# RohanVKashyap/resolution-pde

Hardware: AMD Instinct MI355X
Metric: training samples/sec, FFNO2D NS 256^2 (higher is better)
Workload: dtype f32; 1 GPU; FFNO2D(1,1,width=64,n_layers=4,n_modes=20,factor=4,ff_weight_norm,n_ff_layers=3,layer_norm,dropout=0.1) train step on [B,1,256,256] Gaussian random fields (BASELINE configs[2]); batch_per_gpu=32, global_batch=32, optimizer=AdamW lr=1e-3 (rpde.optim.FlatAdamW: torch.optim.AdamW's rule, one kernel), parallelism=single, grad_bucket_bytes=6828576, target=input advanced by a fixed spectral filter (utils/synthetic.py:advance)

## Files before the change

### resolution-pde_amd/csrc/feedforward.hip

```cpp
#include "rpde_internal.h"
#include "pointwise.h"
#include "gemm_kernel.h"
#include "ff_fused.h"
#include "wgrad_h2.h"
#include "thin_linear.h"
#include "conv_small.h"

#include <vector>

namespace rpde {


static inline int ff_in(const rpde_ff_params* p, int l) { return l == 0 ? p->dim : p->dim * p->factor; }
static inline int ff_out(const rpde_ff_params* p, int l) { return l == p->n_layers - 1 ? p->dim : p->dim * p->factor; }

static inline int wgrad_split(long P, int out_f, int in_f) {
  const int tiles = ((out_f + 127) / 128) * ((in_f + 127) / 128);
  long s = 768 / tiles;
  const long cap = (P + 127) / 128;
  if (s > cap) s = cap;
  if (s < 1) s = 1;
  if (s > 1024) s = 1024;
  return (int)s;
}

static inline bool worth_presplit(long P, int n, int k) { return P >= 1024 && k % 32 == 0 && n > 32; }
static int linear_fwd_impl(const float* x, const float* w, const float* b, float* y, long P, int in_f, int out_f,
                           int act_out, float* dy, float drop_p, uint64_t drop_seed, hipStream_t st,
                           void* wimg = nullptr, const uint64_t* drop_epoch = nullptr, bool wimg_ready = false) {
  if (act_out == RPDE_ACT_IDENTITY && !dy && drop_p == 0.f) {
    if (in_f <= 4 && thin_linear_ok(in_f, out_f) && al16(y)) return thin_expand(x, w, in_f, 1, b, y, P, in_f, out_f, st);
    if (out_f <= 4 && thin_linear_ok(out_f, in_f) && al16(x)) return thin_contract(x, w, in_f, 1, b, y, P, out_f, in_f, st);
  }
  rpde_gemm_desc d = gemm_desc();
  d.A = x; d.a_kmajor = 1; d.lda = in_f;
  d.B = w; d.b_kmajor = 1; d.ldb = in_f;
  if (wimg && worth_presplit(P, out_f, in_f)) {
    if (!wimg_ready) RPDE_TRY(split_weights(w, 1, in_f, out_f, in_f, wimg, st));
    d.b_split = wimg;
  }
  d.C = y; d.ldc = out_f;
  d.M = (int)P; d.N = out_f; d.K = in_f;
  d.bias = b; d.bias_mode = b ? 1 : 0;
  d.write_act = act_out; d.aux_out = act_out ? dy : nullptr;
  if (act_out) { d.drop_p = drop_p; d.drop_seed = drop_seed; d.drop_ld = out_f; d.drop_where = 4; d.drop_epoch = drop_epoch; }
  return launch_gemm(d, st);
}

static int linear_wgrad_impl(const float* x, const float* gy, float* gw, float* gb, long P, int in_f, int out_f,
                             float* ws_slabs, float* ws_colsum, hipStream_t st, int act_x = RPDE_ACT_IDENTITY,
                             FoldJobs* defer = nullptr) {
  if (act_x == RPDE_ACT_IDENTITY && (gw || gb)) {
    if (in_f <= 4 && thin_linear_ok(in_f, out_f) && al16(gy)) return thin_outer(x, gy, gw, 1, gb, nullptr, P, in_f, out_f, ws_slabs, st);
    if (out_f <= 4 && thin_linear_ok(out_f, in_f) && al16(x)) return thin_outer(gy, x, gw, 0, nullptr, gb, P, out_f, in_f, ws_slabs, st);
  }
  if (gw && wgrad_h2_ok(P, out_f, in_f)) {
    RPDE_TRY(wgrad_h2(gy, x, gw, P, in_f, out_f, act_x, ws_slabs, st, defer));
  } else if (gw) {
    const int S = wgrad_split(P, out_f, in_f);
    rpde_gemm_desc d = gemm_desc();
    d.A = gy; d.a_kmajor = 0; d.lda = out_f;
    d.B = x; d.b_kmajor = 0; d.ldb = in_f; d.act_b = act_x;
    d.M = out_f; d.N = in_f; d.K = (int)P;
    if (S > 1) {
      d.C = ws_slabs; d.ldc = in_f; d.ksplit = S; d.sCk = (long)out_f * in_f;
      RPDE_TRY(launch_gemm(d, st));
      if (!(defer && defer->add(ws_slabs, gw, out_f * in_f, S, (long)out_f * in_f)))
        RPDE_TRY(reduce_slabs(ws_slabs, gw, (long)out_f * in_f, S, (long)out_f * in_f, 1.f, 0, st));
    } else {
      d.C = gw; d.ldc = in_f;
      RPDE_TRY(launch_gemm(d, st));
    }
  }
  if (gb) RPDE_TRY(colsum(gy, gb, P, out_f, out_f, ws_colsum, 0, st));
  return RPDE_OK;
}

static inline long colsum_tiles(long P) { return (P + 127) / 128; }
static inline bool can_fuse_colsum(const float* gy, const float* w, const float* gx, const float* z, long P, int in_f,
                                   int out_f) {
  return P > 64 && in_f % 4 == 0 && out_f % 4 == 0 && al16(gy) && al16(w) && al16(gx) && (!z || al16(z));
}

static int linear_dgrad_impl(const float* gy, const float* w, float* gx, long P, int in_f, int out_f,
                             const float* dstored, float* colsum_slab, hipStream_t st, void* wimg = nullptr,
                             bool wimg_ready = false) {
// ... 89 lines not shown
  RPDE_CHECK_ARG(p && prep, "feedforward_prepare: bad arguments");
  Arena ar(prep, prep_bytes);
  const FfFusedImg f(ar);
  RPDE_CHECK_ARG(ff3_fused_ok(p, 32) && ar.ok(), "feedforward_prepare: shape not fused or buffer too small");
  RPDE_CHECK_ARG(p->weights && p->weights[0] && p->weights[1] && p->weights[2], "feedforward_prepare: null weights");
  return ff3_fused_prepare(p, f.img, as_stream(stream));
}

int rpde_feedforward_fwd_prepared(const rpde_ff_params* p, const float* x, const float* residual, float* out, int64_t P,
                                  const void* prep, size_t prep_bytes, void* stream) {
  RPDE_CHECK_ARG(p && x && out && prep && P > 0 && P < (1L << 31), "feedforward_fwd_prepared: bad arguments");
  Arena ar(const_cast<void*>(prep), prep_bytes);
  const FfFusedImg f(ar);
  RPDE_CHECK_ARG(ff3_fused_ok(p, P) && ar.ok(), "feedforward_fwd_prepared: shape not fused");
  RPDE_CHECK_ARG(!p->layer_norm || (p->ln_gamma && p->ln_beta), "feedforward_fwd_prepared: layer_norm needs gamma/beta");
  RPDE_CHECK_ARG(p->dropout_p == 0.f, "feedforward_fwd_prepared: evaluation only");
  return ff3_fused_fwd(p, x, residual, nullptr, nullptr, out , out, P,
                       f.img, as_stream(stream), true);
}

int rpde_feedforward_fwd(const rpde_ff_params* p, const float* x, const float* residual, float* const* hs,
                         float* const* ds, float* z_last, float* out, int64_t P, void* ws, size_t ws_bytes, void* stream) {
  RPDE_CHECK_ARG(p && x && z_last && out && P > 0, "feedforward_fwd: bad arguments");
  RPDE_CHECK_ARG(p->n_layers >= 1 && p->dim > 0 && p->factor > 0, "feedforward_fwd: bad shape");
  RPDE_CHECK_ARG(P < (1L << 31), "feedforward_fwd: too many points for one call");
  RPDE_CHECK_ARG(p->dropout_p >= 0.f && p->dropout_p < 1.f, "feedforward_fwd: dropout %f", p->dropout_p);
  hipStream_t st = as_stream(stream);
  Arena far(ws, ws_bytes);
  const FfFusedImg fused(far);
  if (ff3_fused_ok(p, P) && far.ok()) {
    RPDE_CHECK_ARG(p->weights[0] && p->weights[1] && p->weights[2], "feedforward_fwd: null weights");
    RPDE_CHECK_ARG(!p->layer_norm || (p->ln_gamma && p->ln_beta), "feedforward_fwd: layer_norm needs gamma/beta");
    return ff3_fused_fwd(p, x, residual, hs, ds, z_last, out, P, fused.img, st);
  }
  RPDE_CHECK_ARG(p->n_layers == 1 || hs, "feedforward_fwd: hidden buffers missing");
  const int L = p->n_layers;
  Arena ar(ws, ws_bytes);
  bool all_imgs = ws != nullptr && L <= SplitJobs::MAX;
  const FfFwdImgs imgs(ar, *p, all_imgs ? L : 1);
  all_imgs = all_imgs && ar.ok();
  float* const* wimg = imgs.wimg.data();
  if (all_imgs) {
    SplitJobs sj;
    for (int l = 0; l < L; ++l) {
      RPDE_CHECK_ARG(p->weights[l], "feedforward_fwd: null layer %d weight", l);
      if (worth_presplit(P, ff_out(p, l), ff_in(p, l))) sj.add(p->weights[l], 1, ff_in(p, l), ff_out(p, l), ff_in(p, l), wimg[l]);
    }
    RPDE_TRY(split_weights_multi(sj, st));
  }
  for (int l = 0; l < L; ++l) {
    const bool last = l == L - 1;
    RPDE_CHECK_ARG(p->weights[l] && (last || hs[l]), "feedforward_fwd: null layer %d buffers", l);
    const float* in = l == 0 ? x : hs[l - 1];
    RPDE_TRY(linear_fwd_impl(in, p->weights[l], p->biases ? p->biases[l] : nullptr, last ? z_last : hs[l], P, ff_in(p, l),
                             ff_out(p, l), last ? RPDE_ACT_IDENTITY : RPDE_ACT_GELU, (last || !ds) ? nullptr : ds[l],
                             p->dropout_p, layer_seed(p->seed, l), st, all_imgs ? wimg[l] : wimg[0], p->seed_epoch, all_imgs));
  }
  return ff_tail_fwd(z_last, residual, out, P, p->dim, p->layer_norm, p->ln_eps, p->ln_gamma, p->ln_beta,
                     make_drop(p->dropout_p, layer_seed(p->seed, L - 1), p->seed_epoch), p->post_act, st);
}

int rpde_feedforward_bwd(const rpde_ff_params* p, const float* x, const float* const* hs, const float* const* ds,
                         const float* z_last, const float* grad_out, float* grad_x, float* const* grad_weights,
                         float* const* grad_biases, float* grad_gamma, float* grad_beta, int64_t P, void* ws,
                         size_t ws_bytes, void* stream) {
  RPDE_CHECK_ARG(p && x && z_last && grad_out && P > 0, "feedforward_bwd: bad arguments");
  RPDE_CHECK_ARG(P < (1L << 31), "feedforward_bwd: too many points for one call");
  const int L = p->n_layers;
  const int hid = ff_hid(*p);
  const bool fused = ff3_fused_ok(p, P) && hs && hs[0] && hs[1];
  RPDE_CHECK_ARG(p->n_layers == 1 || (hs && (ds || fused)), "feedforward_bwd: saved hidden tensors missing");
  RPDE_CARVE("feedforward_bwd", FfBwdWork, wk, ws, ws_bytes, *p, P, fused);
  hipStream_t st = as_stream(stream);
  float *buf0 = wk.buf0, *buf1 = wk.buf1, *small = wk.small, *tailws = wk.tailws;
  const std::vector<float*>&slabs_l = wk.slabs, &csum_l = wk.csum, &wt_l = wk.wt;
  void* wt = wt_l[0];

  if (fused) {
    const int recompute = !(ds && ds[0] && ds[1]);
    const int act_h = recompute ? RPDE_ACT_GELU : RPDE_ACT_IDENTITY;
    float *dz3 = wk.dz3, *part = wk.part;
    void* fimg = wk.fimg;
    int grid = 0;
    RPDE_TRY(ff3_fused_bwd_launch(p, recompute ? hs : ds, recompute, z_last, grad_out, dz3, buf0, buf1, nullptr, part, &grid, P,
                                  fimg, st));
    const bool both = grad_x && grad_weights && wgrad_h2_dgrad_ok(P, hid, p->dim);
    if (grad_x && !both) RPDE_TRY(linear_dgrad_impl(buf1, p->weights[0], grad_x, P, p->dim, hid, nullptr, nullptr, st, wt));
    if (grad_weights) {
      FoldJobs folds;
      RPDE_TRY(linear_wgrad_impl(hs[1], dz3, grad_weights[2], nullptr, P, hid, p->dim, slabs_l[2], small, st, act_h, &folds));
      RPDE_TRY(linear_wgrad_impl(hs[0], buf0, grad_weights[1], nullptr, P, hid, hid, slabs_l[1], small, st, act_h, &folds));
      if (both) RPDE_TRY(wgrad_h2_dgrad(buf1, x, p->weights[0], grad_weights[0], grad_x, P, p->dim, hid, slabs_l[0], st, &folds));
      else RPDE_TRY(linear_wgrad_impl(x, buf1, grad_weights[0], nullptr, P, p->dim, hid, slabs_l[0], small, st, RPDE_ACT_IDENTITY, &folds));
      RPDE_TRY(fold_jobs(folds, st));
    }
    {
      ReduceSegs sg;
      memset(&sg, 0, sizeof(sg));
      sg.n = FF3_PART; sg.nseg = 5;
      const int off[5] = {0, 256, 512, 576, 640}, len[5] = {hid, hid, p->dim, p->dim, p->dim};
      float* dst[5] = {grad_biases ? grad_biases[0] : nullptr, grad_biases ? grad_biases[1] : nullptr,
                       grad_biases ? grad_biases[2] : nullptr, p->layer_norm ? grad_gamma : nullptr,
                       p->layer_norm ? grad_beta : nullptr};
      for (int k = 0; k < 5; ++k) { sg.off[k] = off[k]; sg.len[k] = len[k]; sg.dst[k] = dst[k]; }
      RPDE_TRY(reduce_slabs_seg(part, grid, FF3_PART, sg, st));
    }
    return RPDE_OK;
  }

  FoldJobs folds;
  float* dz = buf0;
  float* other = buf1;
  int bias_done = 0;
  RPDE_TRY(ff_tail_bwd(z_last, grad_out, dz, P, p->dim, p->layer_norm, p->ln_eps, p->ln_gamma, p->ln_beta,
                       make_drop(p->dropout_p, layer_seed(p->seed, L - 1), p->seed_epoch), p->post_act, grad_gamma, grad_beta,
                       grad_biases ? grad_biases[L - 1] : nullptr, &bias_done, tailws, st, &folds));
  const bool all_imgs = L <= SplitJobs::MAX;
  if (all_imgs) {
    SplitJobs sj;
    for (int l = grad_x ? 0 : 1; l < L; ++l)
      if (worth_presplit(P, ff_in(p, l), ff_out(p, l))) sj.add(p->weights[l], 0, ff_in(p, l), ff_in(p, l), ff_out(p, l), wt_l[l]);
    RPDE_TRY(split_weights_multi(sj, st));
  }
  for (int l = L - 1; l >= 0; --l) {
    const int in_f = ff_in(p, l), out_f = ff_out(p, l);
    const float* in = l == 0 ? x : hs[l - 1];
    float* gb = (grad_biases && !bias_done) ? grad_biases[l] : nullptr;
    RPDE_TRY(linear_wgrad_impl(in, dz, grad_weights ? grad_weights[l] : nullptr, gb, P, in_f, out_f, slabs_l[l], small, st,
                               RPDE_ACT_IDENTITY, &folds));
    bias_done = 0;
    void* img = all_imgs ? wt_l[l] : wt;
    if (l > 0) {
      RPDE_CHECK_ARG(ds[l - 1], "feedforward_bwd: derivative of layer %d was not saved", l - 1);
      const bool fuse = grad_biases && can_fuse_colsum(dz, p->weights[l], other, ds[l - 1], P, in_f, out_f);
      RPDE_TRY(linear_dgrad_impl(dz, p->weights[l], other, P, in_f, out_f, ds[l - 1], fuse ? csum_l[l] : nullptr, st, img, all_imgs));
      if (fuse) {
        const int S = (int)colsum_tiles(P);
        if (!(S <= 4 * REDUCE_CHUNKS && folds.add(csum_l[l], grad_biases[l - 1], in_f, S, in_f)))
          RPDE_TRY(reduce_slabs_2pass(csum_l[l], grad_biases[l - 1], in_f, S, in_f, csum_l[l] + colsum_tiles(P) * in_f, st));
        bias_done = 1;
      }
      float* t = dz; dz = other; other = t;
    } else if (grad_x) {
      RPDE_TRY(linear_dgrad_impl(dz, p->weights[0], grad_x, P, in_f, out_f, nullptr, nullptr, st, img, all_imgs));
    }
  }
  return fold_jobs(folds, st);
}

struct LinearBwdWork {
  float *slabs, *small;
  LinearBwdWork(Arena& ar, long P, int in_f, int out_f)
      : slabs(ar.take(wgrad_ws_floats(P, in_f, out_f))), small(ar.take(colsum_ws_floats(P, out_f))) {}
};

size_t rpde_linear_ws_bytes(int64_t P, int in_f, int out_f) { return ws_measure<LinearBwdWork>((long)P, in_f, out_f); }

int rpde_linear_fwd(const float* x, const float* w, const float* b, float* out, int64_t P, int in_f, int out_f, void* stream) {
  RPDE_CHECK_ARG(x && w && out && P > 0 && in_f > 0 && out_f > 0 && P < (1L << 31), "linear_fwd: bad arguments");
  return linear_fwd_impl(x, w, b, out, P, in_f, out_f, RPDE_ACT_IDENTITY, nullptr, 0.f, 0, as_stream(stream));
}

int rpde_linear_bwd(const float* x, const float* w, const float* grad_out, float* grad_x, float* grad_w, float* grad_b,
                    int64_t P, int in_f, int out_f, void* ws, size_t ws_bytes, void* stream) {
  RPDE_CHECK_ARG(x && w && grad_out && P > 0 && in_f > 0 && out_f > 0 && P < (1L << 31), "linear_bwd: bad arguments");
  RPDE_CARVE("linear_bwd", LinearBwdWork, wk, ws, ws_bytes, P, in_f, out_f);
  hipStream_t st = as_stream(stream);
  RPDE_TRY(linear_wgrad_impl(x, grad_out, grad_w, grad_b, P, in_f, out_f, wk.slabs, wk.small, st));
  if (grad_x) RPDE_TRY(linear_dgrad_impl(grad_out, w, grad_x, P, in_f, out_f, nullptr, nullptr, st));
  return RPDE_OK;
}
// ... 106 lines not shown
```

### resolution-pde_amd/csrc/ff_fused.h

```cpp
#pragma once
#include "rpde_internal.h"

namespace rpde {
bool ff3_fused_ok(const rpde_ff_params* p, long P);
size_t ff3_fused_ws_floats();
int ff3_fused_prepare(const rpde_ff_params* p, void* ws, hipStream_t st);
int ff3_fused_fwd(const rpde_ff_params* p, const float* x, const float* residual, float* const* hs, float* const* ds,
                  float* z_last, float* out, long P, void* ws, hipStream_t st, bool prepared = false);
constexpr int FF3_PART = 704;
size_t ff3_fused_bwd_part_floats();
int ff3_fused_bwd_launch(const rpde_ff_params* p, const float* const* ds, int recompute, const float* z_last,
                         const float* grad_out, float* dz3, float* du2, float* du1, float* dx, float* part, int* grid_out,
                         long P, void* ws, hipStream_t st);
}
```

### resolution-pde_amd/csrc/ff_fused.hip

```cpp
#include "ff_fused.h"
#include "cw.h"
#include "h2.h"
#include "pointwise.h"

namespace rpde {

#ifdef RPDE_STAMPS
__device__ unsigned long long g_ffstamps[3 * 64];
#define FFSTAMP(i) do { if (stamp_on && stamp_t < 8) g_ffstamps[stamp_w * 64 + stamp_t * 8 + (i)] = __builtin_amdgcn_s_memtime(); } while (0)
__device__ unsigned long long g_fbstamps[3 * 64];
#define FBSTAMP(i) do { if (stamp_on && stamp_t >= 0 && stamp_t < 8) g_fbstamps[stamp_w * 64 + stamp_t * 8 + (i)] = __builtin_amdgcn_s_memtime(); } while (0)
#else
#define FFSTAMP(i) do { } while (0)
#define FBSTAMP(i) do { } while (0)
#endif

constexpr int FF_WAVES = 8;
constexpr int FF_FRAGS = 24;
constexpr int FF_IMG_BYTES = FF_WAVES * FF_FRAGS * 2048;
constexpr int FF_NCONST = 16;
constexpr int FF_PREP_BLOCKS = FF_WAVES * FF_FRAGS * 64 / 1024;

__global__ __launch_bounds__(1024) void k_ff3_prep(const float* __restrict__ w1, const float* __restrict__ w2,
                                                   const float* __restrict__ w3, const float* __restrict__ b1,
// ... 762 lines not shown
}

bool ff3_fused_ok(const rpde_ff_params* p, long P) {
  if (switch_off("RPDE_FUSED_FF")) return false;
  for (int l = 0; l < 3 && p->weights; ++l)
    if (reinterpret_cast<uintptr_t>(p->weights[l]) & 15) return false;
  return p->n_layers == 3 && p->dim == 64 && p->factor == 4 && P >= 32;
}
size_t ff3_fused_ws_floats() { return (FF_IMG_BYTES + FF_NCONST * 4 + 3) / 4; }

int ff3_fused_prepare(const rpde_ff_params* p, void* ws, hipStream_t st) {
  char* img = static_cast<char*>(ws);
  float* consts = reinterpret_cast<float*>(img + FF_IMG_BYTES);
  const float* b1 = p->biases ? p->biases[0] : nullptr;
  const float* b2 = p->biases ? p->biases[1] : nullptr;
  hipLaunchKernelGGL(k_ff3_prep, dim3(FF_PREP_BLOCKS), dim3(1024), 0, st, p->weights[0], p->weights[1], p->weights[2], b1, b2, img, consts);
  RPDE_LAUNCH_CHECK();
  return RPDE_OK;
}

int ff3_fused_fwd(const rpde_ff_params* p, const float* x, const float* residual, float* const* hs, float* const* ds,
                  float* z_last, float* out, long P, void* ws, hipStream_t st, bool prepared) {
  char* img = static_cast<char*>(ws);
  float* consts = reinterpret_cast<float*>(img + FF_IMG_BYTES);
  const float* b1 = p->biases ? p->biases[0] : nullptr;
  const float* b2 = p->biases ? p->biases[1] : nullptr;
  const float* b3 = p->biases ? p->biases[2] : nullptr;
  if (!prepared) RPDE_TRY(ff3_fused_prepare(p, ws, st));
  FF3P A;
  memset(&A, 0, sizeof(A));
  const bool have_h = hs && hs[0] && hs[1], have_d = ds && ds[0] && ds[1];
  const int mode = have_h ? (have_d ? 1 : 2) : 0;
  A.x = x; A.res = residual; A.out = out; A.z3 = z_last;
  if (mode) { A.h1 = hs[0]; A.h2 = hs[1]; }
  if (mode == 1) { A.d1 = ds[0]; A.d2 = ds[1]; }
  A.wimg = img; A.consts = consts; A.b1 = b1; A.b2 = b2; A.b3 = b3; A.gamma = p->ln_gamma; A.beta = p->ln_beta;
  A.P = P; A.layer_norm = p->layer_norm; A.eps = p->ln_eps; A.post_act = p->post_act;
  for (int l = 0; l < 3; ++l) {
    A.drop[l] = make_drop(p->dropout_p, layer_seed(p->seed, l), p->seed_epoch);
  }
  A.ntiles = (int)((P + 31) / 32);
  int cus;
  RPDE_HIP(cu_count(&cus));
  const int grid = A.ntiles < cus ? A.ntiles : cus;
  if (mode == 1) hipLaunchKernelGGL(k_ff3_fwd_h2<1>, dim3(grid), dim3(64 * FF_WAVES), 0, st, A);
  else if (mode == 2) hipLaunchKernelGGL(k_ff3_fwd_h2<2>, dim3(grid), dim3(64 * FF_WAVES), 0, st, A);
  else hipLaunchKernelGGL(k_ff3_fwd_h2<0>, dim3(grid), dim3(64 * FF_WAVES), 0, st, A);
  RPDE_LAUNCH_CHECK();
  return RPDE_OK;
}

size_t ff3_fused_bwd_part_floats() { return (size_t)1024 * FFB_PART; }

int ff3_fused_bwd_launch(const rpde_ff_params* p, const float* const* ds, int recompute, const float* z_last,
                         const float* grad_out, float* dz3, float* du2, float* du1, float* dx, float* part, int* grid_out,
                         long P, void* ws, hipStream_t st) {
  char* img = static_cast<char*>(ws);
  float* consts = reinterpret_cast<float*>(img + FF_IMG_BYTES);
  hipLaunchKernelGGL(k_ff3_prep_bwd, dim3(FF_PREP_BLOCKS), dim3(1024), 0, st, p->weights[0], p->weights[1], p->weights[2], img, consts);
  RPDE_LAUNCH_CHECK();
  FF3B A;
  memset(&A, 0, sizeof(A));
  A.g = grad_out; A.z3 = z_last; A.d1 = ds[0]; A.d2 = ds[1];
  A.dz3 = dz3; A.du2 = du2; A.du1 = du1; A.dx = dx;
  A.wimg = img; A.consts = consts; A.gamma = p->ln_gamma; A.beta = p->ln_beta; A.part = part;
  A.P = P; A.layer_norm = p->layer_norm; A.eps = p->ln_eps; A.post_act = p->post_act;
  DropCfg dc[3];
  for (int l = 0; l < 3; ++l)
    dc[l] = make_drop(p->dropout_p, layer_seed(p->seed, l), p->seed_epoch);
  A.drop0 = dc[0]; A.drop1 = dc[1]; A.drop2 = dc[2];
  A.dmax = 1.13f * A.drop2.scale;
  A.ntiles = (int)((P + 31) / 32);
  int cus;
  RPDE_HIP(cu_count(&cus));
  if (cus > 1024) cus = 1024;
  const int grid = A.ntiles < cus ? A.ntiles : cus;
  if (recompute) hipLaunchKernelGGL(k_ff3_bwd_h2<true>, dim3(grid), dim3(64 * FF_WAVES), 0, st, A);
  else hipLaunchKernelGGL(k_ff3_bwd_h2<false>, dim3(grid), dim3(64 * FF_WAVES), 0, st, A);
  RPDE_LAUNCH_CHECK();
  *grid_out = grid;
  return RPDE_OK;
}

}

#ifdef RPDE_STAMPS
extern "C" int rpde_debug_ffb_stamps(unsigned long long* host_out) {
  RPDE_HIP(hipDeviceSynchronize());
  RPDE_HIP(hipMemcpyFromSymbol(host_out, HIP_SYMBOL(rpde::g_fbstamps), sizeof(unsigned long long) * 3 * 64));
  return RPDE_OK;
}
extern "C" int rpde_debug_ff_stamps(unsigned long long* host_out) {
  RPDE_HIP(hipDeviceSynchronize());
  RPDE_HIP(hipMemcpyFromSymbol(host_out, HIP_SYMBOL(rpde::g_ffstamps), sizeof(unsigned long long) * 3 * 64));
  return RPDE_OK;
}
#endif
```

Baseline: 1043 samples/s.

## Split fused FFN backward into adjoint and layer-1 kernels with fused dgrad/wgrad

When saved dropout/activation derivatives exist, the single fused three-layer backward kernel is replaced by two kernels. The first computes the output-layer adjoint (layer norm, dropout) and the layer-2 input gradient. The second computes the layer-1 input gradient, the first-layer weight-gradient slabs and the bias reduction, so the separate dgrad/wgrad pass for layer 0 is folded in. This is meant to cut the separate layer-0 GEMM passes and improve occupancy, at the cost of writing du2 and dzb to global memory between the two kernels.

After: 1058 samples/s (median of 6 runs). +1.4%, better.

```diff
diff --git a/resolution-pde_amd/csrc/feedforward.hip b/resolution-pde_amd/csrc/feedforward.hip
--- a/resolution-pde_amd/csrc/feedforward.hip
+++ b/resolution-pde_amd/csrc/feedforward.hip
@@ -2,6 +2,7 @@
 #include "pointwise.h"
 #include "gemm_kernel.h"
 #include "ff_fused.h"
+#include "ff_bwd_split.h"
 #include "wgrad_h2.h"
 #include "thin_linear.h"
 #include "conv_small.h"
@@ -257,11 +258,21 @@
     float *dz3 = wk.dz3, *part = wk.part;
     void* fimg = wk.fimg;
     int grid = 0;
-    RPDE_TRY(ff3_fused_bwd_launch(p, recompute ? hs : ds, recompute, z_last, grad_out, dz3, buf0, buf1, nullptr, part, &grid, P,
-                                  fimg, st));
     const bool both = grad_x && grad_weights && wgrad_h2_dgrad_ok(P, hid, p->dim);
+    const bool split = both && !recompute && ff_bwd_split_ok(P, hid, p->dim);
+    if (split) {
+      FoldJobs folds;
+      RPDE_TRY(ff_bwd_split_launch(p, ds, z_last, grad_out, x, dz3, buf0, buf1, grad_x, slabs_l[0], grad_weights[0], part,
+                                   &grid, P, fimg, st, &folds));
+      RPDE_TRY(linear_wgrad_impl(hs[1], dz3, grad_weights[2], nullptr, P, hid, p->dim, slabs_l[2], small, st, act_h, &folds));
+      RPDE_TRY(linear_wgrad_impl(hs[0], buf0, grad_weights[1], nullptr, P, hid, hid, slabs_l[1], small, st, act_h, &folds));
+      RPDE_TRY(fold_jobs(folds, st));
+    } else {
+      RPDE_TRY(ff3_fused_bwd_launch(p, recompute ? hs : ds, recompute, z_last, grad_out, dz3, buf0, buf1, nullptr, part, &grid, P,
+                                    fimg, st));
+    }
     if (grad_x && !both) RPDE_TRY(linear_dgrad_impl(buf1, p->weights[0], grad_x, P, p->dim, hid, nullptr, nullptr, st, wt));
-    if (grad_weights) {
+    if (grad_weights && !split) {
       FoldJobs folds;
       RPDE_TRY(linear_wgrad_impl(hs[1], dz3, grad_weights[2], nullptr, P, hid, p->dim, slabs_l[2], small, st, act_h, &folds));
       RPDE_TRY(linear_wgrad_impl(hs[0], buf0, grad_weights[1], nullptr, P, hid, hid, slabs_l[1], small, st, act_h, &folds));
diff --git a/resolution-pde_amd/csrc/ff_bwd_split.h b/resolution-pde_amd/csrc/ff_bwd_split.h
--- /dev/null
+++ b/resolution-pde_amd/csrc/ff_bwd_split.h
@@ -0,0 +1,13 @@
+#pragma once
+#include "rpde_internal.h"
+#include "pointwise.h"
+
+namespace rpde {
+
+bool ff_bwd_split_ok(long P, int hid, int dim);
+
+int ff_bwd_split_launch(const rpde_ff_params* p, const float* const* ds, const float* z_last, const float* grad_out,
+                        const float* x, float* dz3, float* du2, float* dzb, float* gx, float* slabs, float* gw1, float* part,
+                        int* grid_out, long P, void* fimg, hipStream_t st, FoldJobs* folds);
+
+}
diff --git a/resolution-pde_amd/csrc/ff_bwd_split.hip b/resolution-pde_amd/csrc/ff_bwd_split.hip
--- /dev/null
+++ b/resolution-pde_amd/csrc/ff_bwd_split.hip
@@ -0,0 +1,555 @@
+#include "ff_bwd_split.h"
+#include "ff_fused.h"
+#include "h2.h"
+#include "pointwise.h"
+#include "wgrad_h2.h"
+
+namespace rpde {
+
+constexpr int FS_WAVES = 8;
+constexpr int FS_MAX_GRID = 256;
+struct FsA {
+  const float* g; const float* z3; const float* d2;
+  float* dz3; float* du2; float* dzb;
+  const char* wimg; const float* consts;
+  const float* gamma; const float* beta;
+  float* part;
+  long P; int layer_norm; float eps; int post_act;
+  DropCfg drop2;
+  int ntiles;
+};
+
+constexpr int FA_DZBUF = 0;
+constexpr int FA_VEC = FA_DZBUF + 16384;
+constexpr int FA_ACC = FA_VEC + 512;
+constexpr int FA_INFO = FA_ACC + 7168;
+constexpr int FA_LDS = FA_INFO + 256;
+
+__global__ __launch_bounds__(64 * FS_WAVES, 2) void k_ffs_adjoint(const FsA A0) {
+  __shared__ __attribute__((aligned(16))) char smem[FA_LDS];
+  FsA A = A0;
+  A.drop2 = drop_resolve(A0.drop2);
+  const int tid = threadIdx.x, l = tid & 63, w = tid >> 6, g = l >> 4, li = l & 15;
+  f16x8 w3h[2][2], w3l[2][2];
+  {
+    const char* base = A.wimg + (long)w * FF3_WAVE_IMG + l * 16;
+#pragma unroll
+    for (int f = 0; f < 4; ++f) {
+      w3h[f >> 1][f & 1] = *reinterpret_cast<const f16x8*>(base + f * 2048);
+      w3l[f >> 1][f & 1] = *reinterpret_cast<const f16x8*>(base + f * 2048 + 1024);
+    }
+    float* vecw = reinterpret_cast<float*>(smem + FA_VEC);
+    float* accw = reinterpret_cast<float*>(smem + FA_ACC);
+    for (int i = tid; i < 128; i += 64 * FS_WAVES) vecw[i] = i < 64 ? (A.gamma ? A.gamma[i] : 1.f) : (A.beta ? A.beta[i - 64] : 0.f);
+    for (int i = tid; i < 1792; i += 64 * FS_WAVES) accw[i] = 0.f;
+  }
+  const float* const vec = reinterpret_cast<const float*>(smem + FA_VEC);
+  float* const acc_db2 = reinterpret_cast<float*>(smem + FA_ACC);
+  float* const acc_db3 = acc_db2 + 256;
+  float* const acc_dg = acc_db2 + 768;
+  float* const acc_dbt = acc_db2 + 1280;
+  float* const info = reinterpret_cast<float*>(smem + FA_INFO);
+  const float winv3 = A.consts[2];
+  const int q3 = l >> 4, feat = 4 * li;
+
+  float4 g4n = make_float4(0.f, 0.f, 0.f, 0.f), z4n = g4n, d2n[4];
+  auto issue = [&](int tile) {
+    const long p = min((long)tile * 32 + 4 * w + q3, A.P - 1);
+    g4n = *reinterpret_cast<const float4*>(A.g + p * 64 + feat);
+    z4n = *reinterpret_cast<const float4*>(A.z3 + p * 64 + feat);
+#pragma unroll
+    for (int blk = 0; blk < 2; ++blk)
+#pragma unroll
+      for (int t = 0; t < 2; ++t)
+        d2n[blk * 2 + t] = *reinterpret_cast<const float4*>(A.d2 + min((long)tile * 32 + 16 * blk + li, A.P - 1) * 256 + 16 * (2 * w + t) + 4 * g);
+  };
+#pragma unroll
+  for (int i = 0; i < 4; ++i) d2n[i] = make_float4(0.f, 0.f, 0.f, 0.f);
+  if ((int)blockIdx.x < A.ntiles) issue(blockIdx.x);
+  lds_barrier();
+
+  int par = 0;
+  for (int tile = blockIdx.x; tile < A.ntiles; tile += gridDim.x, par ^= 1) {
+    const int next_tile = tile + gridDim.x;
+    const long p0 = (long)tile * 32;
+    const int ptl = 4 * w + q3;
+    const long pt3 = p0 + ptl;
+    const bool live3 = pt3 < A.P;
+    const long off3 = min(pt3, A.P - 1) * 64 + feat;
+    const float4 g4 = g4n, z4 = z4n;
+    float4 dq[4];
+#pragma unroll
+    for (int i = 0; i < 4; ++i) dq[i] = d2n[i];
+    if (next_tile < A.ntiles) issue(next_tile);
+
+    float s4[4] = {1.f, 1.f, 1.f, 1.f};
+    if (A.drop2.on()) drop_scale4(A.drop2, (uint64_t)(pt3 * 64 + feat), s4);
+    const float tz[4] = {z4.x * s4[0], z4.y * s4[1], z4.z * s4[2], z4.w * s4[3]};
+    float gy[4] = {g4.x, g4.y, g4.z, g4.w};
+    if (!live3) { gy[0] = gy[1] = gy[2] = gy[3] = 0.f; }
+    float dz[4], dzb;
+    float dgm[4] = {0.f, 0.f, 0.f, 0.f}, dbt[4] = {0.f, 0.f, 0.f, 0.f};
+    if (A.layer_norm) {
+      const float mean = row_all16<false>((tz[0] + tz[1]) + (tz[2] + tz[3])) * (1.f / 64.f);
+      const float m2 = row_all16<false>((tz[0] - mean) * (tz[0] - mean) + (tz[1] - mean) * (tz[1] - mean) +
+                                        (tz[2] - mean) * (tz[2] - mean) + (tz[3] - mean) * (tz[3] - mean));
+      const float rstd = rsqrtf(m2 * (1.f / 64.f) + A.eps);
+      const float4 gm = *reinterpret_cast<const float4*>(vec + feat);
+      const float4 bt = *reinterpret_cast<const float4*>(vec + 64 + feat);
+      const float gmv[4] = {gm.x, gm.y, gm.z, gm.w}, btv[4] = {bt.x, bt.y, bt.z, bt.w};
+      float xh[4], dxh[4], s1 = 0.f, s2 = 0.f, am = 0.f;
+#pragma unroll
+      for (int k = 0; k < 4; ++k) {
+        xh[k] = (tz[k] - mean) * rstd;
+        float dy = gy[k];
+        if (A.post_act) dy *= dact_f(A.post_act, xh[k] * gmv[k] + btv[k]);
+        dgm[k] = dy * xh[k];
+        dbt[k] = dy;
+        dxh[k] = dy * gmv[k];
+        s1 += dxh[k];
+        s2 += dxh[k] * xh[k];
+        am = fmaxf(am, fabsf(dxh[k]));
+      }
+      const float S1 = row_all16<false>(s1) * (1.f / 64.f), S2 = row_all16<false>(s2) * (1.f / 64.f);
+      const float AM = row_all16<true>(am);
+#pragma unroll
+      for (int k = 0; k < 4; ++k) dz[k] = rstd * (dxh[k] - S1 - xh[k] * S2) * s4[k];
+      dzb = rstd * (AM + fabsf(S1) + 8.f * fabsf(S2)) * A.drop2.scale;
+    } else {
+      float am = 0.f;
+#pragma unroll
+      for (int k = 0; k < 4; ++k) { dz[k] = gy[k] * dact_f(A.post_act, tz[k]) * s4[k]; am = fmaxf(am, fabsf(dz[k])); }
+      dzb = row_all16<true>(am);
+    }
+    if (live3) *reinterpret_cast<float4*>(A.dz3 + off3) = make_float4(dz[0], dz[1], dz[2], dz[3]);
+    {
+      float b[4];
+#pragma unroll
+      for (int k = 0; k < 4; ++k) {
+        b[k] = live3 ? dz[k] : 0.f;
+        b[k] += lane_xor16(b[k]); b[k] += lane_xor32(b[k]);
+        if (A.layer_norm) {
+          dgm[k] += lane_xor16(dgm[k]); dgm[k] += lane_xor32(dgm[k]);
+          dbt[k] += lane_xor16(dbt[k]); dbt[k] += lane_xor32(dbt[k]);
+        }
+      }
+      if (q3 == 0) {
+        float4* a3 = reinterpret_cast<float4*>(acc_db3 + w * 64 + feat);
+        float4 v3 = *a3;
+        v3.x += b[0]; v3.y += b[1]; v3.z += b[2]; v3.w += b[3];
+        *a3 = v3;
+        if (A.layer_norm) {
+          float4* ag = reinterpret_cast<float4*>(acc_dg + w * 64 + feat);
+          float4* ab = reinterpret_cast<float4*>(acc_dbt + w * 64 + feat);
+          float4 vg = *ag, vb = *ab;
+          vg.x += dgm[0]; vg.y += dgm[1]; vg.z += dgm[2]; vg.w += dgm[3];
+          vb.x += dbt[0]; vb.y += dbt[1]; vb.z += dbt[2]; vb.w += dbt[3];
+          *ag = vg;
+          *ab = vb;
+        }
+      }
+    }
+    {
+      float sdz, sdzi;
+      h2_scale(dzb, 0, sdz, sdzi);
+      uint2 hi, lo;
+      h2_split4(dz[0] * sdz, dz[1] * sdz, dz[2] * sdz, dz[3] * sdz, hi, lo);
+      const int ksz = li >> 3, cz = li & 3;
+      char* dst = smem + FA_DZBUF + par * 8192 + (((ptl >> 4) * 2 + ksz) * 2) * 1024 + (cz * 16 + ((ptl & 15) ^ cz ^ (4 * ksz))) * 16 +
+                  ((li >> 2) & 1) * 8;
+      *reinterpret_cast<uint2*>(dst) = hi;
+      *reinterpret_cast<uint2*>(dst + 1024) = lo;
+      if (li == 0) {
+        info[par * 32 + ptl] = dzb;
+        if (live3) A.dzb[pt3] = dzb;
+      }
+    }
+    lds_barrier();
+
+    float bsum[8] = {0.f, 0.f, 0.f, 0.f, 0.f, 0.f, 0.f, 0.f};
+#pragma unroll
+    for (int blk = 0; blk < 2; ++blk) {
+      const int zu = (l & 48) | ((l & 15) ^ (l >> 4));
+      const char* zb = smem + FA_DZBUF + par * 8192 + (blk * 2) * 2048;
+      const f16x8 zh0 = *reinterpret_cast<const f16x8*>(zb + zu * 16), zl0 = *reinterpret_cast<const f16x8*>(zb + 1024 + zu * 16);
+      const f16x8 zh1 = *reinterpret_cast<const f16x8*>(zb + 2048 + (zu ^ 4) * 16), zl1 = *reinterpret_cast<const f16x8*>(zb + 3072 + (zu ^ 4) * 16);
+      const long pt = p0 + 16 * blk + li;
+      float sz, inv_a;
+      h2_scale(info[par * 32 + blk * 16 + li], 0, sz, inv_a);
+      inv_a *= winv3;
+#pragma unroll
+      for (int t = 0; t < 2; ++t) {
+        f32x4v acc = {0.f, 0.f, 0.f, 0.f};
+        acc = h2_mfma32(w3h[t][0], w3l[t][0], zh0, zl0, acc);
+        acc = h2_mfma32(w3h[t][1], w3l[t][1], zh1, zl1, acc);
+        const int hid = 16 * (2 * w + t) + 4 * g;
+        const float4 d = dq[blk * 2 + t];
+        float u[4] = {acc[0] * inv_a * d.x, acc[1] * inv_a * d.y, acc[2] * inv_a * d.z, acc[3] * inv_a * d.w};
+#pragma unroll
+        for (int r = 0; r < 4; ++r) pin(u[r]);
+        if (pt < A.P) {
+          *reinterpret_cast<float4*>(A.du2 + pt * 256 + hid) = make_float4(u[0], u[1], u[2], u[3]);
+#pragma unroll
+          for (int r = 0; r < 4; ++r) bsum[4 * t + r] += u[r];
+        }
+      }
+    }
+#pragma unroll
+    for (int i = 0; i < 8; ++i) bsum[i] = row_sum15(bsum[i]);
+    if (li == 15) {
+#pragma unroll
+      for (int i = 0; i < 8; ++i) acc_db2[16 * (2 * w + (i >> 2)) + 4 * g + (i & 3)] += bsum[i];
+    }
+  }
+  lds_barrier();
+  {
+    float* part = A.part + (long)blockIdx.x * FF3_PART;
+    for (int i = 256 + tid; i < FF3_PART; i += 64 * FS_WAVES) {
+      float v;
+      if (i < 512) v = acc_db2[i - 256];
+      else {
+        const float* a8 = acc_db3 + ((i - 512) >> 6) * 512 + ((i - 512) & 63);
+        v = 0.f;
+#pragma unroll
+        for (int ww = 0; ww < FS_WAVES; ++ww) v += a8[ww * 64];
+      }
+      part[i] = v;
+    }
+  }
+}
+
+struct FsB {
+  const float* du2; const float* d1; const float* x; const float* dzb; const float* w1;
+  float* gx; float* slabs; float* part;
+  const char* wimg; const float* consts;
+  long P; float dmax; int ntiles;
+};
+
+constexpr int FL_PANEL = 8192;
+constexpr int FL_DUBUF = 0;
+constexpr int FL_PAN = FL_DUBUF + 32768;
+constexpr int FL_X = FL_PAN + 4 * FL_PANEL;
+constexpr int FL_W1 = FL_X + FL_PANEL;
+constexpr int FL_LDS = FL_W1 + 65536;
+
+__global__ __launch_bounds__(64 * FS_WAVES, 2) void k_ffs_layer1(const FsB A) {
+  __shared__ __attribute__((aligned(16))) char smem[FL_LDS];
+  __shared__ int einfo[FS_WAVES];
+  __shared__ float xmax[FS_WAVES];
+  __shared__ float wmax[FS_WAVES];
+  __shared__ float acc_db1[256];
+  const int tid = threadIdx.x, l = tid & 63, w = tid >> 6, g = l >> 4, li = l & 15;
+  f16x8 w2h[2][8], w2l[2][8];
+  {
+    const char* base = A.wimg + (long)w * FF3_WAVE_IMG + l * 16;
+#pragma unroll
+    for (int f = 0; f < 16; ++f) {
+      w2h[f >> 3][f & 7] = *reinterpret_cast<const f16x8*>(base + (4 + f) * 2048);
+      w2l[f >> 3][f & 7] = *reinterpret_cast<const f16x8*>(base + (4 + f) * 2048 + 1024);
+    }
+  }
+  if (tid < 256) acc_db1[tid] = 0.f;
+  char* const wfrag = smem + FL_W1;
+  float w_inv = 1.f;
+  {
+    constexpr int NF = 8 * 4 * 64 / (64 * FS_WAVES);
+    float wv[NF][8];
+    float m = 0.f;
+#pragma unroll
+    for (int r = 0; r < NF; ++r) {
+      const int c = tid + r * 64 * FS_WAVES, fl = c & 63, nt = (c >> 6) & 3, ks = c >> 8;
+#pragma unroll
+      for (int j = 0; j < 8; ++j) {
+        wv[r][j] = A.w1[(long)(32 * ks + 8 * (fl >> 4) + j) * 64 + 16 * nt + (fl & 15)];
+        m = fmaxf(m, fabsf(wv[r][j]));
+      }
+    }
+    m = wave_max(m);
+    if (l == 0) wmax[w] = m;
+    __syncthreads();
+    m = 0.f;
+#pragma unroll
+    for (int i = 0; i < FS_WAVES; ++i) m = fmaxf(m, wmax[i]);
+    float w_scale;
+    h2_scale(m, 0, w_scale, w_inv);
+#pragma unroll
+    for (int r = 0; r < NF; ++r) {
+      const int c = tid + r * 64 * FS_WAVES, fl = c & 63, nt = (c >> 6) & 3, ks = c >> 8;
+      uint2 h0, l0, h1, l1;
+      h2_split4(wv[r][0] * w_scale, wv[r][1] * w_scale, wv[r][2] * w_scale, wv[r][3] * w_scale, h0, l0);
+      h2_split4(wv[r][4] * w_scale, wv[r][5] * w_scale, wv[r][6] * w_scale, wv[r][7] * w_scale, h1, l1);
+      char* d = wfrag + (ks * 4 + nt) * 2048 + fl * 16;
+      *reinterpret_cast<uint4*>(d) = make_uint4(h0.x, h0.y, h1.x, h1.y);
+      *reinterpret_cast<uint4*>(d + 1024) = make_uint4(l0.x, l0.y, l1.x, l1.y);
+    }
+  }
+  const float winv2 = A.consts[1], c3t = A.consts[3];
+
+  const int xrow = tid >> 4, xc = tid & 15;
+  float4 du2r[4], d1r[4], xr;
+  float bzr[2];
+  const unsigned cb = 32 * w + 4 * g;
+  auto load_du2 = [&](int tile) {
+    const long t0 = (long)tile * 32;
+    const int rmax = (int)min(31L, A.P - 1 - t0);
+    const float* __restrict__ src = A.du2 + t0 * 256;
+    const float* __restrict__ bz = A.dzb + t0;
+#pragma unroll
+    for (int blk = 0; blk < 2; ++blk) {
+      const unsigned r = (unsigned)min(16 * blk + li, rmax);
+      bzr[blk] = bz[r];
+#pragma unroll
+      for (int t = 0; t < 2; ++t) du2r[blk * 2 + t] = *reinterpret_cast<const float4*>(src + (r * 256u + cb + 16u * t));
+    }
+  };
+  auto load_d1 = [&](int tile) {
+    const long t0 = (long)tile * 32;
+    const int rmax = (int)min(31L, A.P - 1 - t0);
+    const float* __restrict__ src = A.d1 + t0 * 256;
+#pragma unroll
+    for (int blk = 0; blk < 2; ++blk) {
+      const unsigned r = (unsigned)min(16 * blk + li, rmax);
+#pragma unroll
+      for (int t = 0; t < 2; ++t) d1r[blk * 2 + t] = *reinterpret_cast<const float4*>(src + (r * 256u + cb + 16u * t));
+    }
+  };
+  auto load_x = [&](int tile) {
+    const long t0 = (long)tile * 32;
+    const float* __restrict__ src = A.x + t0 * 64;
+    xr = t0 + xrow < A.P ? *reinterpret_cast<const float4*>(src + (unsigned)(xrow * 64 + 4 * xc)) : make_float4(0.f, 0.f, 0.f, 0.f);
+  };
+
+  const int wm = w >> 1, wn = w & 1;
+  typedef s16x4v __attribute__((address_space(3))) * lds_tr;
+  f32x4v gw[4][2];
+#pragma unroll
+  for (int i = 0; i < 4; ++i)
+#pragma unroll
+    for (int j = 0; j < 2; ++j) gw[i][j] = (f32x4v){0.f, 0.f, 0.f, 0.f};
+  int ea_used[2] = {15, 15}, eb_used = 15;
+  int e_run = 15, e_x = 15;
+  const int dg_mt = w & 1, dg_nt = w >> 1;
+
+  if ((int)blockIdx.x < A.ntiles) { load_du2(blockIdx.x); load_d1(blockIdx.x); load_x(blockIdx.x); }
+  lds_barrier();
+
+  for (int tile = blockIdx.x; tile < A.ntiles; tile += gridDim.x) {
+    const int next_tile = tile + gridDim.x;
+    const bool has_next = next_tile < A.ntiles;
+    const long p0 = (long)tile * 32;
+    float inv_b[2];
+#pragma unroll
+    for (int blk = 0; blk < 2; ++blk) {
+      float s_du2, ai;
+      h2_scale(c3t * bzr[blk] * A.dmax, 0, s_du2, ai);
+      inv_b[blk] = ai * winv2;
+      const float4 a = du2r[blk * 2], b = du2r[blk * 2 + 1];
+      const float hv[8] = {a.x * s_du2, a.y * s_du2, a.z * s_du2, a.w * s_du2, b.x * s_du2, b.y * s_du2, b.z * s_du2, b.w * s_du2};
+      h2_put_frag(smem + FL_DUBUF + ((blk * 8 + w) * 2) * 1024 + l * 16, hv);
+    }
+    {
+      float m = fmaxf(fmaxf(fabsf(xr.x), fabsf(xr.y)), fmaxf(fabsf(xr.z), fabsf(xr.w)));
+      m = wave_max(m);
+      if (l == 0) xmax[w] = m;
+    }
+    lds_barrier();
+
+    float u[4][4];
+    float bsum[8] = {0.f, 0.f, 0.f, 0.f, 0.f, 0.f, 0.f, 0.f};
+    {
+      f32x4v acc[2][2];
+#pragma unroll
+      for (int blk = 0; blk < 2; ++blk) {
+        acc[blk][0] = (f32x4v){0.f, 0.f, 0.f, 0.f}; acc[blk][1] = (f32x4v){0.f, 0.f, 0.f, 0.f};
+#pragma unroll
+        for (int kap = 0; kap < 8; ++kap) {
+          const char* hb = smem + FL_DUBUF + ((blk * 8 + kap) * 2) * 1024 + l * 16;
+          const f16x8 bh = *reinterpret_cast<const f16x8*>(hb), bl = *reinterpret_cast<const f16x8*>(hb + 1024);
+          acc[blk][0] = h2_mfma32(w2h[0][kap], w2l[0][kap], bh, bl, acc[blk][0]);
+          acc[blk][1] = h2_mfma32(w2h[1][kap], w2l[1][kap], bh, bl, acc[blk][1]);
+        }
+      }
+#pragma unroll
+      for (int blk = 0; blk < 2; ++blk) {
+        const bool live = p0 + 16 * blk + li < A.P;
+#pragma unroll
+        for (int t = 0; t < 2; ++t) {
+          const float4 d4 = d1r[blk * 2 + t];
+          const float d[4] = {d4.x, d4.y, d4.z, d4.w};
+          float* v = u[blk * 2 + t];
+          float s[4];
+#pragma unroll
+          for (int r = 0; r < 4; ++r) { s[r] = acc[blk][t][r] * inv_b[blk]; v[r] = s[r] * d[r]; }
+          if (live) {
+#pragma unroll
+            for (int r = 0; r < 4; ++r) bsum[4 * t + r] = __builtin_fmaf(s[r], d[r], bsum[4 * t + r]);
+          } else {
+            v[0] = v[1] = v[2] = v[3] = 0.f;
+          }
+        }
+      }
+    }
+    if (has_next) { load_du2(next_tile); load_d1(next_tile); }
+#pragma unroll
+    for (int i = 0; i < 8; ++i) bsum[i] = row_sum15(bsum[i]);
+    if (li == 15) {
+#pragma unroll
+      for (int i = 0; i < 8; ++i) acc_db1[16 * (2 * w + (i >> 2)) + 4 * g + (i & 3)] += bsum[i];
+    }
+    {
+      float m = 0.f;
+#pragma unroll
+      for (int i = 0; i < 4; ++i) m = fmaxf(fmaxf(m, fmaxf(fabsf(u[i][0]), fabsf(u[i][1]))), fmaxf(fabsf(u[i][2]), fabsf(u[i][3])));
+      m = wave_max(m);
+      e_run = max(e_run, (int)(__float_as_uint(m) >> 23) & 0xff);
+      e_run = min(e_run, 254);
+      const float scale = __uint_as_float((unsigned)(268 - e_run) << 23);
+      char* const dst = smem + FL_PAN + (w >> 1) * FL_PANEL;
+#pragma unroll
+      for (int blk = 0; blk < 2; ++blk)
+#pragma unroll
+        for (int t = 0; t < 2; ++t) {
+          const float* v = u[blk * 2 + t];
+          uint2 hi, lo;
+          h2_split4(v[0] * scale, v[1] * scale, v[2] * scale, v[3] * scale, hi, lo);
+          const int off = stage_off(16 * blk + li, (w & 1) * 8 + 4 * t + g);
+          *reinterpret_cast<uint2*>(dst + off) = hi;
+          *reinterpret_cast<uint2*>(dst + 4096 + off) = lo;
+        }
+      if (l == 0) einfo[w] = e_run;
+    }
+    {
+      float m = 0.f;
+#pragma unroll
+      for (int i = 0; i < FS_WAVES; ++i) m = fmaxf(m, xmax[i]);
+      e_x = max(e_x, (int)(__float_as_uint(m) >> 23) & 0xff);
+      e_x = min(e_x, 254);
+      const float scale = __uint_as_float((unsigned)(268 - e_x) << 23);
+      uint2 hi, lo;
+      h2_split4(xr.x * scale, xr.y * scale, xr.z * scale, xr.w * scale, hi, lo);
+      const int off = stage_off(xrow, xc);
+      *reinterpret_cast<uint2*>(smem + FL_X + off) = hi;
+      *reinterpret_cast<uint2*>(smem + FL_X + 4096 + off) = lo;
+    }
+    if (has_next) load_x(next_tile);
+    lds_barrier();
+
+    int lc = l;
+    asm volatile("" : "+v"(lc));
+    const int gc = lc >> 4, lic = lc & 15;
+    {
+      const int q = lic >> 2, pp = lic & 3;
+      const int tsw = ((q >> 1) & 1) | ((gc & 1) << 1);
+      const int trow = (8 * gc + q) * 128 + pp * 8;
+      auto frag = [&](const char* panel, int tile, f16x8& hi, f16x8& lo) {
+        const char* t = panel + trow + ((tile ^ tsw) << 5);
+        union { struct { s16x4v a, b; } h; f16x8 v; } uh, ul;
+        uh.h.a = __builtin_amdgcn_ds_read_tr16_b64_v4i16((lds_tr)(t));
+        uh.h.b = __builtin_amdgcn_ds_read_tr16_b64_v4i16((lds_tr)(t + 512));
+        ul.h.a = __builtin_amdgcn_ds_read_tr16_b64_v4i16((lds_tr)(t + 4096));
+        ul.h.b = __builtin_amdgcn_ds_read_tr16_b64_v4i16((lds_tr)(t + 4096 + 512));
+        hi = uh.v; lo = ul.v;
+      };
+      const int eb = __builtin_amdgcn_readfirstlane(e_x);
+#pragma unroll
+      for (int k = 0; k < 2; ++k) {
+        const int ea = __builtin_amdgcn_readfirstlane(einfo[2 * wm + k]);
+        if (ea + eb != ea_used[k] + eb_used) {
+          const int d = (ea_used[k] + eb_used) - (ea + eb);
+          const float f = d > -126 ? __uint_as_float((unsigned)(127 + d) << 23) : 0.f;
+#pragma unroll
+          for (int j = 0; j < 2; ++j) { gw[2 * k][j] *= f; gw[2 * k + 1][j] *= f; }
+        }
+        ea_used[k] = ea;
+      }
+      eb_used = eb;
+      f16x8 bh[2], bl[2];
+#pragma unroll
+      for (int j = 0; j < 2; ++j) frag(smem + FL_X, 2 * wn + j, bh[j], bl[j]);
+#pragma unroll
+      for (int i = 0; i < 4; ++i) {
+        f16x8 ah, al;
+        frag(smem + FL_PAN + wm * FL_PANEL, i, ah, al);
+#pragma unroll
+        for (int j = 0; j < 2; ++j) gw[i][j] = h2_mfma32(ah, al, bh[j], bl[j], gw[i][j]);
+      }
+    }
+    {
+      f32x4v tot = (f32x4v){0.f, 0.f, 0.f, 0.f};
+      const int row = 16 * dg_mt + lic;
+#pragma unroll
+      for (int hp = 0; hp < 8; ++hp) {
+        const char* pa_ = smem + FL_PAN + (hp >> 1) * FL_PANEL + stage_off(row, 2 * (4 * (hp & 1) + gc));
+        const f16x8 ah = *reinterpret_cast<const f16x8*>(pa_), al = *reinterpret_cast<const f16x8*>(pa_ + 4096);
+        const char* wb = wfrag + (hp * 4 + dg_nt) * 2048 + lc * 16;
+        const f16x8 bh = *reinterpret_cast<const f16x8*>(wb), bl = *reinterpret_cast<const f16x8*>(wb + 1024);
+        const f32x4v part = h2_mfma32(ah, al, bh, bl, (f32x4v){0.f, 0.f, 0.f, 0.f});
+        const int ek = __builtin_amdgcn_readfirstlane(einfo[hp]);
+        const float fk = __uint_as_float((unsigned)(ek - 14) << 23) * w_inv;
+        tot += part * fk;
+      }
+      float t0 = tot[0], t1 = tot[1], t2 = tot[2], t3 = tot[3];
+      quad_transpose(t0, t1, t2, t3);
+      const int rq = 16 * dg_mt + 4 * gc + (lic & 3);
+      if (p0 + rq < A.P) *reinterpret_cast<float4*>(A.gx + p0 * 64 + (unsigned)(rq * 64 + 16 * dg_nt + 4 * (lic >> 2))) = make_float4(t0, t1, t2, t3);
+    }
+  }
+
+  const float fb = __uint_as_float((unsigned)(eb_used - 14) << 23);
+  float* __restrict__ out = A.slabs + (long)blockIdx.x * 256 * 64;
+  const unsigned o0 = (unsigned)((wm * 64 + 4 * g) * 64 + wn * 32 + li);
+#pragma unroll
+  for (int i = 0; i < 4; ++i) {
+    const float fa = __uint_as_float((unsigned)(ea_used[i >> 1] - 14) << 23);
+#pragma unroll
+    for (int j = 0; j < 2; ++j)
+#pragma unroll
+      for (int r = 0; r < 4; ++r) out[o0 + (unsigned)((16 * i + r) * 64 + 16 * j)] = gw[i][j][r] * fa * fb;
+  }
+  lds_barrier();
+  if (tid < 256) A.part[(long)blockIdx.x * FF3_PART + tid] = acc_db1[tid];
+}
+
+bool ff_bwd_split_ok(long P, int hid, int dim) { return !switch_off("RPDE_FF_BWD_SPLIT") && wgrad_h2_dgrad_ok(P, hid, dim); }
+
+int ff_bwd_split_launch(const rpde_ff_params* p, const float* const* ds, const float* z_last, const float* grad_out,
+                        const float* x, float* dz3, float* du2, float* dzb, float* gx, float* slabs, float* gw1, float* part,
+                        int* grid_out, long P, void* fimg, hipStream_t st, FoldJobs* folds) {
+  RPDE_CHECK_ARG(ff_bwd_split_ok(P, p->dim * p->factor, p->dim) && ds && ds[0] && ds[1] && gx && gw1 && slabs,
+                 "ff_bwd_split: unsupported call");
+  const char* img;
+  const float* consts;
+  RPDE_TRY(ff3_fused_bwd_prepare(p, fimg, &img, &consts, st));
+  const int ntiles = (int)((P + 31) / 32);
+  int cus;
+  RPDE_HIP(cu_count(&cus));
+  int grid = cus < FS_MAX_GRID ? cus : FS_MAX_GRID;
+  if (ntiles < grid) grid = ntiles;
+  const DropCfg drop2 = make_drop(p->dropout_p, layer_seed(p->seed, 2), p->seed_epoch);
+
+  FsA a;
+  memset(&a, 0, sizeof(a));
+  a.g = grad_out; a.z3 = z_last; a.d2 = ds[1];
+  a.dz3 = dz3; a.du2 = du2; a.dzb = dzb;
+  a.wimg = img; a.consts = consts; a.gamma = p->ln_gamma; a.beta = p->ln_beta; a.part = part;
+  a.P = P; a.layer_norm = p->layer_norm; a.eps = p->ln_eps; a.post_act = p->post_act;
+  a.drop2 = drop2; a.ntiles = ntiles;
+  hipLaunchKernelGGL(k_ffs_adjoint, dim3(grid), dim3(64 * FS_WAVES), 0, st, a);
+  RPDE_LAUNCH_CHECK();
+
+  FsB b;
+  memset(&b, 0, sizeof(b));
+  b.du2 = du2; b.d1 = ds[0]; b.x = x; b.dzb = dzb; b.w1 = p->weights[0];
+  b.gx = gx; b.slabs = slabs; b.part = part;
+  b.wimg = img; b.consts = consts;
+  b.P = P; b.dmax = 1.13f * drop2.scale;
+  b.ntiles = ntiles;
+  hipLaunchKernelGGL(k_ffs_layer1, dim3(grid), dim3(64 * FS_WAVES), 0, st, b);
+  RPDE_LAUNCH_CHECK();
+  *grid_out = grid;
+  const int hid = p->dim * p->factor;
+  if (folds && folds->add(slabs, gw1, hid * p->dim, grid, (long)hid * p->dim)) return RPDE_OK;
+  return reduce_slabs(slabs, gw1, (long)hid * p->dim, grid, (long)hid * p->dim, 1.f, 0, st);
+}
+
+}
diff --git a/resolution-pde_amd/csrc/ff_fused.h b/resolution-pde_amd/csrc/ff_fused.h
--- a/resolution-pde_amd/csrc/ff_fused.h
+++ b/resolution-pde_amd/csrc/ff_fused.h
@@ -12,4 +12,6 @@
 int ff3_fused_bwd_launch(const rpde_ff_params* p, const float* const* ds, int recompute, const float* z_last,
                          const float* grad_out, float* dz3, float* du2, float* du1, float* dx, float* part, int* grid_out,
                          long P, void* ws, hipStream_t st);
+constexpr int FF3_WAVE_IMG = 24 * 2048;
+int ff3_fused_bwd_prepare(const rpde_ff_params* p, void* ws, const char** img, const float** consts, hipStream_t st);
 }
diff --git a/resolution-pde_amd/csrc/ff_fused.hip b/resolution-pde_amd/csrc/ff_fused.hip
--- a/resolution-pde_amd/csrc/ff_fused.hip
+++ b/resolution-pde_amd/csrc/ff_fused.hip
@@ -868,6 +868,16 @@
   return RPDE_OK;
 }
 
+static_assert(FF3_WAVE_IMG == FF_FRAGS * 2048, "ff_fused.h states the image layout");
+int ff3_fused_bwd_prepare(const rpde_ff_params* p, void* ws, const char** img_out, const float** consts_out, hipStream_t st) {
+  char* img = static_cast<char*>(ws);
+  float* consts = reinterpret_cast<float*>(img + FF_IMG_BYTES);
+  hipLaunchKernelGGL(k_ff3_prep_bwd, dim3(FF_PREP_BLOCKS), dim3(1024), 0, st, p->weights[0], p->weights[1], p->weights[2], img, consts);
+  RPDE_LAUNCH_CHECK();
+  *img_out = img; *consts_out = consts;
+  return RPDE_OK;
+}
+
 }
 
 #ifdef RPDE_STAMPS
```
